# wavelab/libwave

Hardware: AMD Instinct MI355X
Metric: point-cloud registrations/sec (1M<->1M pts, ICP) (higher is better)
Workload: dtype f32

## Files before the change

libwave_amd/csrc/wm_nn.hip:

```cpp
#include "wm_nn_scan.hpp"

namespace wm {

template <int STATS, bool BAL, bool COST = false>
__global__ void __launch_bounds__(64) __attribute__((amdgpu_waves_per_eu(5, 5)))
    k_nn_grid(const LevelsDev *__restrict__ lv, const float4 *__restrict__ src, unsigned n,
              IcpDevState *__restrict__ st, float thr_d2, unsigned long long *__restrict__ keys,
              float4 *__restrict__ match_pt, const float4 *__restrict__ tgt_orig,
              float r_light_cells, float lane_lf, float coop_lf, float r0_cells, unsigned chunk_sz,
              double *__restrict__ partials, unsigned *__restrict__ cost_out,
              unsigned long long *__restrict__ phase_out, long long *__restrict__ bins) {
    const unsigned lane = threadIdx.x & 63u;
    const unsigned row = chunk_sz ? xcd_remap_chunked(blockIdx.x, chunk_sz) : xcd_remap(blockIdx.x, gridDim.x);
    const unsigned i = row * 64u + lane;
    const bool active = i < n;
    const unsigned ic = min(i, n - 1u);
    const float4 p_e = src[ic];
    const unsigned long long prev_e = keys[ic];
    const float4 tp_e = match_pt[ic];
    if (st->done) return;
    unsigned cost = 0;
    unsigned long long prof[3] = {0ull, 0ull, 0ull};
    const unsigned long long prof_start = COST ? clock64() : 0ull;
    __shared__ uint2 s_runs[BAL ? 1 : kRowChunk * 64];
    __shared__ BalHolder<BAL> s_hold;
    const int L = lv->n;
    const int L_levels = L;
    float hl[kMaxLevels];
#pragma unroll
    for (int k = 0; k < kMaxLevels; ++k) hl[k] = lv->g[k < L ? k : 0].h;
    const float h0 = hl[0];
    const float rmax = sqrtf(thr_d2) * 1.0001f + 1e-6f;
    const float r_light = r_light_cells * h0;
    const bool have_prev = st->have_prev != 0;
    float qx = 0.f, qy = 0.f, qz = 0.f, r = 0.f;
    float bqx = 0.f, bqy = 0.f, bqz = 0.f;
    unsigned long long best = make_key(thr_d2, kNoIdx);
    unsigned long long seeded = best;
    bool heavy = false;
    bool mine = active;
    unsigned long long prev = ~0ull;
    float4 tp = make_float4(0.f, 0.f, 0.f, 0.f);
    if (active) {
        if (have_prev) {
            prev = prev_e;
            tp = tp_e;
        }
        xform(st->Tf, p_e, qx, qy, qz);
        if (st->slab_on && !(qx >= st->slab_lo && qx < st->slab_hi)) mine = false;
    }
    if (mine) {
        r = r0_cells * h0;
        if (prev != ~0ull) {
            const unsigned pidx = (unsigned) prev;
            r = rmax;
            if (pidx != kNoIdx) {
                const float d2b = canon_d2(qx, qy, qz, tp);
                if (d2b <= thr_d2) {
                    best = seeded = make_key(d2b, pidx);
                    bqx = tp.x;
                    bqy = tp.y;
                    bqz = tp.z;
                    r = fmaxf(sqrtf(d2b) * 1.0001f + 1e-6f, 0.05f * h0);
                }
            }
        }
        r = fminf(r, rmax);
        heavy = r > r_light;
    }
    const unsigned long long prof_pro = COST ? clock64() : 0ull;
    if constexpr (BAL) {
        BalLds &L = s_hold.v;
        L.q[lane] = make_float4(qx, qy, qz, 0.f);
        L.seeded[lane] = seeded;
        L.bq[0][lane] = bqx;
        L.bq[1][lane] = bqy;
        L.bq[2][lane] = bqz;
        asm volatile("" ::: "memory");
        bool live = mine && !heavy;
        for (int pass = 0; pass < 32 && __ballot(live) != 0ull; ++pass) {
            const int l = nn_level_for(hl, L_levels, lane_lf, r);
            const unsigned long long lv_mask = __ballot(live);
            const int l0 = __builtin_amdgcn_readlane(l, __ffsll((long long) lv_mask) - 1);
            float margin;
            if (__ballot(live && l != l0) == 0ull) {
                const GridDev g = lv->g[l0];
                best = scan_box_bal<COST, kBalRowChunk>(g, live, qx, qy, qz, r, best, &margin, L, lane, have_prev, g.pts, cost, prof);
            } else {
                const GridDev g = lv->g[l];
                L.base[lane] = (unsigned long long) g.pts;
                best = scan_box_bal<COST, kBalRowChunk>(g, live, qx, qy, qz, r, best, &margin, L, lane, have_prev, nullptr, cost, prof);
            }
            if (live) {
                if constexpr (COST) cost += 1u << 24;
                const float bd2 = __uint_as_float((unsigned) (best >> 32));
                if (nn_certified(margin, bd2, thr_d2)) {
                    live = false;
                } else {
                    r = nn_grow_radius(best, bd2, r, rmax);
                    heavy = r > r_light;
                    live = !heavy;
                }
            }
        }
    } else if (mine) {
        for (int pass = 0; !heavy && pass < 32; ++pass) {
            int l = 0;
            while (l < L - 1 && lv->g[l].h < lane_lf * r) ++l;
            const GridDev g = lv->g[l];
            float margin;
            best = scan_box<COST>(g, qx, qy, qz, r, best, &margin, s_runs, lane, have_prev, cost);
            if constexpr (COST) cost += 1u << 24;
            const float bd2 = __uint_as_float((unsigned) (best >> 32));
            if (nn_certified(margin, bd2, thr_d2)) break;
            r = nn_grow_radius(best, bd2, r, rmax);
            heavy = r > r_light;
        }
    }
    const unsigned long long prof_pass = COST ? clock64() : 0ull;
    unsigned long long todo = __ballot(heavy);
    const unsigned n_heavy = __popcll(todo);
    float seed = 0.f;
    while (todo) {
        const int sl = __ffsll((long long) todo) - 1;
        todo &= todo - 1;
        const float ux = rl_f(qx, sl), uy = rl_f(qy, sl), uz = rl_f(qz, sl);
        float ur = rl_f(r, sl);
        unsigned long long ub = ((unsigned long long) rl_u((unsigned) (best >> 32), sl) << 32) |
                                rl_u((unsigned) best, sl);
        if ((unsigned) ub == kNoIdx && seed > ur) ur = fminf(seed, rmax);
        for (int pass = 0; pass < 64; ++pass) {
            int l = 0;
            while (l < L - 1 && lv->g[l].h < coop_lf * ur) ++l;
            const GridDev g = lv->g[l];
            float margin;
            ub = coop_scan_box(g, ux, uy, uz, ur, ub, lane, &margin);
            const float bd2 = __uint_as_float((unsigned) (ub >> 32));
            if (nn_certified(margin, bd2, thr_d2)) break;
            if (ur >= rmax) break;
            ur = nn_grow_radius(ub, bd2, ur, rmax);
        }
        seed = ((unsigned) ub != kNoIdx) ? 1.25f * sqrtf(__uint_as_float((unsigned) (ub >> 32))) : ur;
        if ((int) lane == sl) best = ub;
    }
    const unsigned lane_e = __builtin_amdgcn_mbcnt_hi(~0u, __builtin_amdgcn_mbcnt_lo(~0u, 0u));
    const unsigned i_e = BAL ? row * 64u + lane_e : i;
    if constexpr (BAL) {
        asm volatile("" ::: "memory");
        BalLds &L = s_hold.v;
        seeded = L.seeded[lane_e];
        bqx = L.bq[0][lane_e];
        bqy = L.bq[1][lane_e];
        bqz = L.bq[2][lane_e];
    }
    if (mine) {
        st_u64(&keys[i_e], best);
        if (best != seeded && (unsigned) best != kNoIdx) {
            const f4v c = ((gp_f4) tgt_orig)[(unsigned) best];
            bqx = c.x;
            bqy = c.y;
            bqz = c.z;
        }
        if (!(best == seeded && (unsigned) best != kNoIdx))
            st_f4(&match_pt[i_e], bqx, bqy, bqz, __uint_as_float((unsigned) best));
    }
    if (lane == 0 && n_heavy) atomicAdd(&st->queue_count[1], n_heavy);
    const unsigned long long prof_store = COST ? clock64() : 0ull;
    if constexpr (COST) {
        if (active) cost_out[i_e] = mine ? (cost | (heavy ? 0x80000000u : 0u)) : 0u;
    }
    if constexpr (STATS >= 0) {
        double a[kAcc];
        icp_terms<STATS>(a, mine, (unsigned) best != kNoIdx, qx, qy, qz, bqx, bqy, bqz,
                         __uint_as_float((unsigned) (best >> 32)),
                         (unsigned) best != (unsigned) seeded && (i_e & st->changed_mask) == 0u);
        acc_halve<kAcc, 32>(a, lane);
        const int comp = acc_comp_of_lane(lane);
        if (comp >= 0) {
            if (bins) bins_add(bins, row % (unsigned) kBinCount, (unsigned) comp, a[0]);
            else st_f64(&partials[(size_t) row * kAcc + comp], a[0]);
        }
    }
    if constexpr (COST) {
        if (lane_e == 0 && phase_out) {
            const unsigned long long t_end = clock64();
            atomicAdd(&phase_out[0], prof[0]);
            atomicAdd(&phase_out[1], prof[1]);
            atomicAdd(&phase_out[2], prof[2]);
            atomicAdd(&phase_out[3], prof_pro - prof_start);
            atomicAdd(&phase_out[4], prof_pass - prof_pro);
            atomicAdd(&phase_out[5], prof_store - prof_pass);
            atomicAdd(&phase_out[6], t_end - prof_store);
            atomicAdd(&phase_out[7], 1ull);
        }
    }
}

constexpr int kBruteTile = 1024;

__global__ void __launch_bounds__(kBlock) k_init_keys(unsigned long long *keys, unsigned n,
                                                       const IcpDevState *st, float thr_d2) {
    if (st->done) return;
    const unsigned i = blockIdx.x * kBlock + threadIdx.x;
    if (i < n) keys[i] = make_key(thr_d2, kNoIdx);
}

__global__ void __launch_bounds__(kBlock)
    k_nn_brute(const float4 *__restrict__ tgt, unsigned m, const float4 *__restrict__ src,
               unsigned n, const IcpDevState *__restrict__ st, float thr_d2,
               unsigned long long *__restrict__ keys) {
    if (st->done) return;
    __shared__ float4 tile[kBruteTile];
    const unsigned i = blockIdx.x * kBlock + threadIdx.x;
    const unsigned per = (m + gridDim.y - 1) / gridDim.y;
    const unsigned m0 = blockIdx.y * per, m1 = min(m0 + per, m);
    float qx = 0, qy = 0, qz = 0;
    if (i < n) xform(st->Tf, src[i], qx, qy, qz);
    const bool mine = !(st->slab_on && !(qx >= st->slab_lo && qx < st->slab_hi));
    unsigned long long best = make_key(thr_d2, kNoIdx);
    for (unsigned t0 = m0; t0 < m1; t0 += kBruteTile) {
        const unsigned cnt = min((unsigned) kBruteTile, m1 - t0);
        __syncthreads();
        for (unsigned k = threadIdx.x; k < cnt; k += kBlock) tile[k] = tgt[t0 + k];
        __syncthreads();
        for (unsigned k = 0; k < cnt; ++k) {
            const float4 t = tile[k];
            const unsigned long long key = make_key(canon_d2(qx, qy, qz, t), __float_as_uint(t.w));
            best = key < best ? key : best;
        }
    }
    if (i < n && mine && best < make_key(thr_d2, kNoIdx)) atomicMin(&keys[i], best);
}

__global__ void __launch_bounds__(kBlock)
    k_fill_match(const unsigned long long *__restrict__ keys, unsigned n,
                 const float4 *__restrict__ tgt, const IcpDevState *__restrict__ st,
                 float4 *__restrict__ match_pt) {
    if (st->done) return;
    const unsigned i = blockIdx.x * kBlock + threadIdx.x;
    if (i >= n) return;
    const unsigned idx = (unsigned) keys[i];
    match_pt[i] = idx == kNoIdx ? make_float4(0.f, 0.f, 0.f, __uint_as_float(kNoIdx)) : tgt[idx];
}

static float threshold_below(double max_corr, bool strict) {
    const double m2 = max_corr * max_corr;
    if (!(m2 < 3.0e38)) return 3.0e38f;
    float f = (float) m2;
    if (strict ? (double) f >= m2 : (double) f > m2) f = nextafterf(f, 0.0f);
    return f;
}
float threshold_d2(double max_corr) { return threshold_below(max_corr, false); }
float threshold_d2_strict(double max_corr) { return threshold_below(max_corr, true); }

int nn_sums_target(wm_ctx *ctx, int stats_mode, bool use_bins, unsigned blocks, long long **bins, unsigned *rows_out) {
    *bins = nullptr;
    if (stats_mode >= 0 && use_bins) {
        if (!ctx->bins.p) return WM_ERR_STATE;
        *bins = ctx->bins.as<long long>();
    } else if (stats_mode >= 0) {
        WM_HIP(ctx, ctx->partials.reserve((size_t) blocks * kAcc * sizeof(double)));
        if (rows_out) *rows_out = blocks;
    }
    return WM_OK;
}

template <int STATS, bool BAL, bool COST = false>
static void launch_nn_grid_t(wm_ctx *ctx, unsigned blocks, float thr_d2, unsigned xcd_chunk, long long *bins = nullptr) {
    hipLaunchKernelGGL(HIP_KERNEL_NAME(k_nn_grid<STATS, BAL, COST>), dim3(blocks), dim3(64), 0, ctx->stream,
                       ctx->d_levels.as<LevelsDev>(), ctx->src_sorted.as<float4>(), (unsigned) ctx->n_src,
                       ctx->d_state.as<IcpDevState>(), thr_d2, ctx->keys.as<unsigned long long>(),
                       ctx->match_pt.as<float4>(), ctx->tgt_orig.as<float4>(), ctx->tune_r_light,
                       ctx->tune_lane_lf, ctx->tune_coop_lf, ctx->tune_r0, xcd_chunk, ctx->partials.as<double>(),
                       ctx->cost_log.p ? ctx->cost_log.as<unsigned>() + (size_t) ctx->cost_log_iter * ctx->n_src : nullptr,
                       ctx->phase_log.p ? ctx->phase_log.as<unsigned long long>() + 8 * (size_t) ctx->cost_log_iter : nullptr, bins);
}

int launch_nn_grid(wm_ctx *ctx, float thr_d2, hipEvent_t ev0, hipEvent_t ev1, hipEvent_t ev2,
                   int stats_mode, unsigned *rows_out, bool use_bins) {
    const unsigned n = (unsigned) ctx->n_src;
    if (rows_out) *rows_out = 0;
    if (n == 0) return WM_OK;
    unsigned blocks = (n + 63u) / 64u;
    blocks = (blocks + 7u) & ~7u;
    unsigned xcd_chunk = 0;
    if (ctx->tune_xcd_chunk > 0 && blocks >= 32u * (unsigned) ctx->tune_xcd_chunk) {
        xcd_chunk = (unsigned) ctx->tune_xcd_chunk;
        const unsigned m = 8u * xcd_chunk;
        blocks = (blocks + m - 1u) / m * m;
    }
    long long *bins = nullptr;
    const int rc = nn_sums_target(ctx, stats_mode, use_bins, blocks, &bins, rows_out);
    if (rc != WM_OK) return rc;
    const bool bal = ctx->tune_nn_balanced && ctx->n_tgt_input < (1u << 26) - 8u;
    if (ev0) WM_HIP(ctx, hipEventRecord(ev0, ctx->stream));
    if (stats_mode == WM_ICP_SVD && ctx->cost_log.p && ctx->cost_log_iter < ctx->cost_log_cap) {
        if (bal) launch_nn_grid_t<WM_ICP_SVD, true, true>(ctx, blocks, thr_d2, xcd_chunk, bins);
        else launch_nn_grid_t<WM_ICP_SVD, false, true>(ctx, blocks, thr_d2, xcd_chunk, bins);
        ctx->cost_log_iter++;
    } else if (stats_mode < 0) {
        if (bal) launch_nn_grid_t<-1, true>(ctx, blocks, thr_d2, xcd_chunk);
        else launch_nn_grid_t<-1, false>(ctx, blocks, thr_d2, xcd_chunk);
    } else if (stats_mode == WM_ICP_SVD) {
        if (bal) launch_nn_grid_t<WM_ICP_SVD, true>(ctx, blocks, thr_d2, xcd_chunk, bins);
        else launch_nn_grid_t<WM_ICP_SVD, false>(ctx, blocks, thr_d2, xcd_chunk, bins);
    } else {
        if (bal) launch_nn_grid_t<WM_ICP_GN6, true>(ctx, blocks, thr_d2, xcd_chunk, bins);
        else launch_nn_grid_t<WM_ICP_GN6, false>(ctx, blocks, thr_d2, xcd_chunk, bins);
    }
    if (ev1) WM_HIP(ctx, hipEventRecord(ev1, ctx->stream));
    if (ev2) WM_HIP(ctx, hipEventRecord(ev2, ctx->stream));
    WM_HIP(ctx, hipGetLastError());
    return WM_OK;
}

int launch_nn_brute(wm_ctx *ctx, float thr_d2, hipEvent_t ev0, hipEvent_t ev1) {
    const unsigned n = (unsigned) ctx->n_src, m = (unsigned) ctx->n_tgt_input;
    if (n == 0) return WM_OK;
    const IcpDevState *st = ctx->d_state.as<IcpDevState>();
    unsigned long long *keys = ctx->keys.as<unsigned long long>();
    const unsigned bx = (n + kBlock - 1) / kBlock;
    unsigned splits = 1;
    if (m > 0) {
        splits = (2048 + bx - 1) / bx;
        const unsigned max_splits = (m + kBruteTile - 1) / kBruteTile;
        if (splits > max_splits) splits = max_splits;
        if (splits < 1) splits = 1;
    }
    if (ev0) WM_HIP(ctx, hipEventRecord(ev0, ctx->stream));
    hipLaunchKernelGGL(k_init_keys, dim3(bx), dim3(kBlock), 0, ctx->stream, keys, n, st, thr_d2);
    if (m > 0)
        hipLaunchKernelGGL(k_nn_brute, dim3(bx, splits), dim3(kBlock), 0, ctx->stream,
                           ctx->tgt_orig.as<float4>(), m, ctx->src_sorted.as<float4>(), n, st,
                           thr_d2, keys);
    hipLaunchKernelGGL(k_fill_match, dim3(bx), dim3(kBlock), 0, ctx->stream, keys, n,
                       ctx->tgt_orig.as<float4>(), st, ctx->match_pt.as<float4>());
    if (ev1) WM_HIP(ctx, hipEventRecord(ev1, ctx->stream));
    WM_HIP(ctx, hipGetLastError());
    return WM_OK;
}

}
```

libwave_amd/csrc/wm_nn_scan.hpp:

```cpp
#pragma once
#include "wm_internal.hpp"
#include "wm_icp_step.hpp"
#include "wm_bins.hpp"
#include "wm_wave.hpp"

namespace wm {

__device__ __forceinline__ unsigned long long make_key(float d2, unsigned idx) {
    return ((unsigned long long) __float_as_uint(d2) << 32) | idx;
}

__device__ __forceinline__ float canon_d2(float qx, float qy, float qz, const float4 &t) {
    const float dx = qx - t.x, dy = qy - t.y, dz = qz - t.z;
    return __fadd_rn(__fadd_rn(__fmul_rn(dx, dx), __fmul_rn(dy, dy)), __fmul_rn(dz, dz));
}

__device__ __forceinline__ void xform(const float *T, const float4 &p, float &x, float &y,
                                      float &z) {
    x = __fadd_rn(__fadd_rn(__fadd_rn(__fmul_rn(T[0], p.x), __fmul_rn(T[1], p.y)),
                            __fmul_rn(T[2], p.z)), T[3]);
    y = __fadd_rn(__fadd_rn(__fadd_rn(__fmul_rn(T[4], p.x), __fmul_rn(T[5], p.y)),
                            __fmul_rn(T[6], p.z)), T[7]);
    z = __fadd_rn(__fadd_rn(__fadd_rn(__fmul_rn(T[8], p.x), __fmul_rn(T[9], p.y)),
                            __fmul_rn(T[10], p.z)), T[11]);
}

__device__ __forceinline__ unsigned xcd_remap(unsigned b, unsigned nblocks) {
    const unsigned per = (nblocks + 7u) / 8u;
    return (b & 7u) * per + (b >> 3);
}
__device__ __forceinline__ unsigned xcd_remap_chunked(unsigned b, unsigned S) {
    const unsigned x = b & 7u, l = b >> 3;
    const unsigned chunk = l / S;
    return (chunk * 8u + x) * S + (l - chunk * S);
}

typedef float f4v __attribute__((ext_vector_type(4)));
typedef const __attribute__((address_space(1))) f4v *gp_f4;
typedef const __attribute__((address_space(1))) unsigned *gp_u32;
__device__ __forceinline__ float4 ldp(const float4 *p, size_t j) {
    const f4v v = ((gp_f4) p)[j];
    return make_float4(v.x, v.y, v.z, v.w);
}
__device__ __forceinline__ unsigned ldc(const unsigned *p, size_t j) { return ((gp_u32) p)[j]; }
__device__ __forceinline__ void st_f4(float4 *p, float x, float y, float z, float w) {
    f4v v = {x, y, z, w};
    __builtin_nontemporal_store(v, (f4v *) p);
}
__device__ __forceinline__ void st_u64(unsigned long long *p, unsigned long long v) { __builtin_nontemporal_store(v, p); }
__device__ __forceinline__ void st_f64(double *p, double v) { __builtin_nontemporal_store(v, p); }
__device__ __forceinline__ float canon_d2v(float qx, float qy, float qz, const f4v &t) {
    return canon_d2(qx, qy, qz, make_float4(t.x, t.y, t.z, t.w));
}

__device__ __forceinline__ unsigned long long scan_run(const float4 *__restrict__ pts, unsigned s,
                                                       unsigned e, float qx, float qy, float qz,
                                                       unsigned long long best) {
    for (unsigned j = s; j < e; j += 4) {
        const gp_f4 p = (gp_f4) pts + j;
        const f4v t0 = p[0], t1 = p[1], t2 = p[2], t3 = p[3];
        const unsigned long long k0 = make_key(canon_d2v(qx, qy, qz, t0), __float_as_uint(t0.w));
        const unsigned long long k1 = make_key(canon_d2v(qx, qy, qz, t1), __float_as_uint(t1.w));
        const unsigned long long k2 = make_key(canon_d2v(qx, qy, qz, t2), __float_as_uint(t2.w));
        const unsigned long long k3 = make_key(canon_d2v(qx, qy, qz, t3), __float_as_uint(t3.w));
        const unsigned long long a = k0 < k1 ? k0 : k1, b = k2 < k3 ? k2 : k3;
        const unsigned long long m = a < b ? a : b;
        best = m < best ? m : best;
    }
    return best;
}

constexpr int kRowChunk = 6;
constexpr int kLayeredRows = 18;
template <bool COST>
__device__ __forceinline__ unsigned long long scan_box(const GridDev &g, float qx, float qy,
                                                       float qz, float r, unsigned long long best,
                                                       float *margin, uint2 *runs, unsigned lane,
                                                       bool allow_layered, unsigned &cost) {
    const float big = 4.0e6f;
    const float fx = fminf(fmaxf((qx - g.ox) * g.inv_h, -big), big);
    const float fy = fminf(fmaxf((qy - g.oy) * g.inv_h, -big), big);
    const float fz = fminf(fmaxf((qz - g.oz) * g.inv_h, -big), big);
    const float rc = r * g.inv_h + g.slack;
    const int x0 = (int) floorf(fx - rc), x1 = (int) floorf(fx + rc);
    const int y0 = (int) floorf(fy - rc), y1 = (int) floorf(fy + rc);
    const int z0 = (int) floorf(fz - rc), z1 = (int) floorf(fz + rc);
    const float mx = fminf(fx - (float) x0, (float) (x1 + 1) - fx);
    const float my = fminf(fy - (float) y0, (float) (y1 + 1) - fy);
    const float mz = fminf(fz - (float) z0, (float) (z1 + 1) - fz);
    *margin = (fminf(mx, fminf(my, mz)) - g.slack) * g.h;
    const int xa = max(x0, 0), xb = min(x1, g.nx - 1);
    const int ya = max(y0, 0), yb = min(y1, g.ny - 1);
    const int za = max(z0, 0), zb = min(z1, g.nz - 1);
    if (xa > xb || ya > yb || za > zb) return best;
    auto lookup_and_walk = [&](const unsigned (&a0)[kRowChunk], const unsigned (&a1)[kRowChunk]) {
        unsigned rs[kRowChunk], re[kRowChunk];
#pragma unroll
        for (int u = 0; u < kRowChunk; ++u) {
            rs[u] = ldc(g.cell_start, a0[u]);
            re[u] = ldc(g.cell_start, a1[u]);
        }
        unsigned cnt = 0;
        if constexpr (COST) cost += 1u << 16;
#pragma unroll
        for (int u = 0; u < kRowChunk; ++u)
            if (re[u] > rs[u]) runs[cnt++ * 64u + lane] = make_uint2(rs[u], re[u]);
        unsigned idx = 0, j = 0, e = 0;
        if (cnt) {
            const uint2 run = runs[lane];
            j = run.x;
            e = run.y;
        }
        while (j < e) {
            const gp_f4 p = (gp_f4) g.pts + j;
            const f4v t0 = p[0], t1 = p[1], t2 = p[2], t3 = p[3];
            const unsigned long long k0 = make_key(canon_d2v(qx, qy, qz, t0), __float_as_uint(t0.w));
            const unsigned long long k1 = make_key(canon_d2v(qx, qy, qz, t1), __float_as_uint(t1.w));
            const unsigned long long k2 = make_key(canon_d2v(qx, qy, qz, t2), __float_as_uint(t2.w));
            const unsigned long long k3 = make_key(canon_d2v(qx, qy, qz, t3), __float_as_uint(t3.w));
            const unsigned long long a = k0 < k1 ? k0 : k1, b = k2 < k3 ? k2 : k3;
            const unsigned long long m = a < b ? a : b;
            best = m < best ? m : best;
            j += 4;
            if constexpr (COST) cost += 1u;
            if (j >= e && ++idx < cnt) {
                const uint2 run = runs[idx * 64u + lane];
                j = run.x;
                e = run.y;
            }
        }
    };
    const bool layered =
        allow_layered && __popcll(__ballot((yb - ya + 1) * (zb - za + 1) > kLayeredRows)) >= 8;
    if (layered) {
        for (int kz = 0;; ++kz) {
            const int zz = za + kz;
            const bool zact = zz <= zb;
            if (__ballot(zact) == 0ull) break;
            const float Rb =
                __builtin_amdgcn_sqrtf(__uint_as_float((unsigned) (best >> 32))) * g.inv_h * 1.00001f;
            const float lim = Rb + g.slack;
            const float lim2 = lim * lim, c0 = Rb * Rb + 2.f * g.slack * lim;
            const float rz = fmaxf(fmaxf((float) zz - fz, fz - (float) (zz + 1)), 0.f);
            const float rz2 = rz * rz;
            const float hy = __builtin_amdgcn_sqrtf(fmaxf(lim2 - rz2, 0.f)) * 1.00001f;
            const bool zin = zact && !(rz2 > lim2);
            const int yl = zin ? max(ya, __float2int_rd(fy - hy)) : 1;
            const int yh = zin ? min(yb, __float2int_rd(fy + hy)) : 0;
            const unsigned basez = (unsigned) zz * g.ny * g.nx;
            for (int y0 = yl; __ballot(y0 <= yh) != 0ull; y0 += kRowChunk) {
                unsigned a0[kRowChunk], a1[kRowChunk];
#pragma unroll
                for (int u = 0; u < kRowChunk; ++u) {
                    const int yy = y0 + u;
                    const float yf = (float) yy;
                    const float ry = fmaxf(fmaxf(yf - fy, fy - (yf + 1.f)), 0.f);
                    const float rho2 = ry * ry + rz2;
                    const float hx = __builtin_amdgcn_sqrtf(fmaxf(c0 - rho2, 0.f)) * 1.00001f + g.slack;
                    const int xl = max(xa, __float2int_rd(fx - hx)), xh = min(xb, __float2int_rd(fx + hx));
                    const bool ok = yy <= yh && !(rho2 > lim2) && xl <= xh;
                    const unsigned base = basez + (unsigned) yy * g.nx;
                    a0[u] = ok ? base + xl : 0u;
                    a1[u] = ok ? base + xh + 1 : 0u;
                }
                lookup_and_walk(a0, a1);
            }
        }
        return best;
    }
    int yy = ya, zz = za;
    while (zz <= zb) {
        const float Rb =
            __builtin_amdgcn_sqrtf(__uint_as_float((unsigned) (best >> 32))) * g.inv_h * 1.00001f;
        const float lim = Rb + g.slack;
        const float lim2 = lim * lim, c0 = Rb * Rb + 2.f * g.slack * lim;
        unsigned a0[kRowChunk], a1[kRowChunk];
#pragma unroll
        for (int u = 0; u < kRowChunk; ++u) {
            const float ry = fmaxf(fmaxf((float) yy - fy, fy - (float) (yy + 1)), 0.f);
            const float rz = fmaxf(fmaxf((float) zz - fz, fz - (float) (zz + 1)), 0.f);
            const float rho2 = ry * ry + rz * rz;
            const float hx = __builtin_amdgcn_sqrtf(fmaxf(c0 - rho2, 0.f)) * 1.00001f + g.slack;
            const int xl = max(xa, __float2int_rd(fx - hx)), xh = min(xb, __float2int_rd(fx + hx));
            const bool ok = zz <= zb && !(rho2 > lim2) && xl <= xh;
            const unsigned base = ((unsigned) zz * g.ny + yy) * g.nx;
            a0[u] = ok ? base + xl : 0u;
            a1[u] = ok ? base + xh + 1 : 0u;
            const bool wrap = yy >= yb;
            yy = wrap ? ya : yy + 1;
            zz += wrap;
        }
        lookup_and_walk(a0, a1);
    }
    return best;
}

__device__ __forceinline__ unsigned long long scan_run_bound(const float4 *__restrict__ pts, unsigned s, unsigned e,
                                                             float qx, float qy, float qz, unsigned long long best,
                                                             unsigned &second) {
    for (unsigned j = s; j < e; j += 4) {
        const gp_f4 p = (gp_f4) pts + j;
        const f4v t[4] = {p[0], p[1], p[2], p[3]};
#pragma unroll
        for (int u = 0; u < 4; ++u) {
            const unsigned long long k = make_key(canon_d2v(qx, qy, qz, t[u]), __float_as_uint(t[u].w));
            if (k < best) {
                second = min(second, (unsigned) (best >> 32));
                best = k;
            } else if (k != best) {
                second = min(second, (unsigned) (k >> 32));
            }
        }
    }
    return best;
}

__device__ __forceinline__ unsigned long long wave_min_u64(unsigned long long v) {
#pragma unroll
    for (int off = 32; off > 0; off >>= 1) {
        const unsigned long long o = __shfl_xor(v, off);
        v = o < v ? o : v;
    }
    return v;
}

__device__ __forceinline__ float rl_f(float v, int lane) {
    return __int_as_float(__builtin_amdgcn_readlane(__float_as_int(v), lane));
}
__device__ __forceinline__ unsigned rl_u(unsigned v, int lane) {
    return (unsigned) __builtin_amdgcn_readlane((int) v, lane);
}

constexpr int kBalCap = 1024;
constexpr int kBalRowChunk = 3;
struct BalLds {
    unsigned items[kBalCap + 1];
    float4 q[64];
    unsigned long long base[64];
    unsigned long long best[64];
    unsigned long long seeded[64];
    float bq[3][64];
};

__device__ __forceinline__ unsigned wave_incl_scan(unsigned v) {
    v += (unsigned) __builtin_amdgcn_update_dpp(0, (int) v, 0x111, 0xf, 0xf, true);
    v += (unsigned) __builtin_amdgcn_update_dpp(0, (int) v, 0x112, 0xf, 0xf, true);
    v += (unsigned) __builtin_amdgcn_update_dpp(0, (int) v, 0x114, 0xf, 0xf, true);
    v += (unsigned) __builtin_amdgcn_update_dpp(0, (int) v, 0x118, 0xf, 0xf, true);
    v += (unsigned) __builtin_amdgcn_update_dpp(0, (int) v, 0x142, 0xa, 0xf, false);
    v += (unsigned) __builtin_amdgcn_update_dpp(0, (int) v, 0x143, 0xc, 0xf, false);
    return v;
}

template <bool B>
struct BalHolder {
    BalLds v;
};
template <>
struct BalHolder<false> {
    int unused;
};

struct Bound {
    unsigned second;
    float pad;
    unsigned *lds;
    float4 *win;
    bool ok;
    __device__ __forceinline__ float prune_r(unsigned long long best) const {
        const float b = __builtin_amdgcn_sqrtf(__uint_as_float((unsigned) (best >> 32))) * 1.00001f + pad;
        return fminf(b, __builtin_amdgcn_sqrtf(__uint_as_float(second)) * 1.00001f);
    }
};

template <bool BOUND>
__device__ __forceinline__ void pooled_rounds(BalLds &L, const unsigned *items, unsigned T, unsigned lane,
                                              const float4 *ubase, Bound *bnd) {
    for (unsigned k0 = 0; k0 < T; k0 += 64u) {
        const unsigned k = k0 + lane;
        if (k < T) {
            const unsigned it = items[k];
            const unsigned owner = it >> 26, j = it & 0x3FFFFFFu;
            const float4 q = L.q[owner];
            const gp_f4 p = (gp_f4) (ubase ? ubase : (const float4 *) L.base[owner]) + j;
            const f4v t0 = p[0], t1 = p[1], t2 = p[2], t3 = p[3];
            const float d0 = canon_d2v(q.x, q.y, q.z, t0), d1 = canon_d2v(q.x, q.y, q.z, t1);
            const float d2 = canon_d2v(q.x, q.y, q.z, t2), d3 = canon_d2v(q.x, q.y, q.z, t3);
            const unsigned m = min(min(__float_as_uint(d0), __float_as_uint(d1)), min(__float_as_uint(d2), __float_as_uint(d3)));
            if (m <= __float_as_uint(q.w)) {
                const unsigned long long k0_ = make_key(d0, __float_as_uint(t0.w)), k1_ = make_key(d1, __float_as_uint(t1.w));
                const unsigned long long k2_ = make_key(d2, __float_as_uint(t2.w)), k3_ = make_key(d3, __float_as_uint(t3.w));
                const unsigned long long a = k0_ < k1_ ? k0_ : k1_, b = k2_ < k3_ ? k2_ : k3_;
                if constexpr (BOUND) {
                    const unsigned long long mn = a < b ? a : b;
                    const unsigned u0 = __float_as_uint(d0), u1 = __float_as_uint(d1), u2 = __float_as_uint(d2),
                                   u3 = __float_as_uint(d3);
                    const unsigned lo01 = min(u0, u1), hi01 = max(u0, u1), lo23 = min(u2, u3), hi23 = max(u2, u3);
                    const unsigned sec = min(max(lo01, lo23), min(hi01, hi23));
                    const unsigned long long old = atomicMin(&L.best[owner], mn);
                    unsigned push = sec;
                    if (old != mn) push = min(push, (unsigned) ((old > mn ? old : mn) >> 32));
                    atomicMin(&bnd->lds[owner], push);
                    if (old > mn && bnd->win) {
                        const f4v c = mn == k0_ ? t0 : (mn == k1_ ? t1 : (mn == k2_ ? t2 : t3));
                        bnd->win[owner] = make_float4(c.x, c.y, c.z, c.w);
                    }
                } else {
                    atomicMin(&L.best[owner], a < b ? a : b);
                }
            }
        }
    }
}

template <bool COST, int RC, bool BOUND = false>
__device__ __forceinline__ void balanced_walk(BalLds &L, const unsigned (&rs)[RC],
                                              const unsigned (&re)[RC], unsigned lane,
                                              const float4 *pts, const float4 *ubase, float qx, float qy,
                                              float qz, unsigned long long &best, unsigned &cost,
                                              unsigned long long *prof, Bound *bnd = nullptr) {
    const unsigned long long prof_t0 = COST ? clock64() : 0ull;
    unsigned len[RC], t = 0, longest = 0;
#pragma unroll
    for (int u = 0; u < RC; ++u) {
        len[u] = (unsigned) max((int) (re[u] - rs[u]), 0);
        t += (len[u] + 3u) >> 2;
        longest = max(longest, len[u]);
    }
    const unsigned incl = wave_incl_scan(t);
    const unsigned T = rl_u(incl, 63);
    if (T == 0u) return;
    if constexpr (COST) cost += t;
    if (T > (unsigned) kBalCap) {
        if constexpr (BOUND) {
#pragma unroll
            for (int u = 0; u < RC; ++u) best = scan_run_bound(pts, rs[u], re[u], qx, qy, qz, best, bnd->second);
        } else {
#pragma unroll
            for (int u = 0; u < RC; ++u) best = scan_run(pts, rs[u], re[u], qx, qy, qz, best);
        }
        return;
    }
    unsigned off = incl - t;
    const unsigned tag = lane << 26;
    if (__ballot(longest > 8u) == 0ull) {
#pragma unroll
        for (int u = 0; u < RC; ++u) {
            L.items[len[u] > 0u ? off : (unsigned) kBalCap] = tag | rs[u];
            L.items[len[u] > 4u ? off + 1u : (unsigned) kBalCap] = tag | (rs[u] + 4u);
            off += (len[u] + 3u) >> 2;
        }
    } else {
#pragma unroll
        for (int u = 0; u < RC; ++u)
            for (unsigned j = rs[u]; j < re[u]; j += 4u) L.items[off++] = tag | j;
    }
    L.best[lane] = best;
    if constexpr (BOUND) {
        const float pr = bnd->prune_r(best);
        bnd->lds[lane] = bnd->second;
        reinterpret_cast<unsigned *>(&L.q[lane])[3] = __float_as_uint(pr * pr);
    } else {
        reinterpret_cast<unsigned *>(&L.q[lane])[3] = (unsigned) (best >> 32);
    }
    __builtin_amdgcn_wave_barrier();
    pooled_rounds<BOUND>(L, L.items, T, lane, ubase, bnd);
    __builtin_amdgcn_wave_barrier();
    best = L.best[lane];
    if constexpr (BOUND) bnd->second = bnd->lds[lane];
    if constexpr (COST) {
        prof[0] += clock64() - prof_t0;
        prof[1] += (T + 63u) / 64u;
        prof[2] += 1;
    }
}

template <bool COST, int RC, bool BOUND = false>
__device__ __forceinline__ unsigned long long scan_box_bal(const GridDev &g, bool live, float qx, float qy,
                                                           float qz, float r, unsigned long long best,
                                                           float *margin, BalLds &L, unsigned lane,
                                                           bool allow_layered, const float4 *ubase,
                                                           unsigned &cost, unsigned long long *prof, Bound *bnd = nullptr) {
    const float big = 4.0e6f;
    const float fx = fminf(fmaxf((qx - g.ox) * g.inv_h, -big), big);
    const float fy = fminf(fmaxf((qy - g.oy) * g.inv_h, -big), big);
    const float fz = fminf(fmaxf((qz - g.oz) * g.inv_h, -big), big);
    const float rc = r * g.inv_h + g.slack;
    const int x0 = (int) floorf(fx - rc), x1 = (int) floorf(fx + rc);
    const int y0 = (int) floorf(fy - rc), y1 = (int) floorf(fy + rc);
    const int z0 = (int) floorf(fz - rc), z1 = (int) floorf(fz + rc);
    const float mx = fminf(fx - (float) x0, (float) (x1 + 1) - fx);
    const float my = fminf(fy - (float) y0, (float) (y1 + 1) - fy);
    const float mz = fminf(fz - (float) z0, (float) (z1 + 1) - fz);
    *margin = (fminf(mx, fminf(my, mz)) - g.slack) * g.h;
    const int xa = max(x0, 0), xb = min(x1, g.nx - 1);
    const int ya = max(y0, 0), yb = min(y1, g.ny - 1);
    const int za = max(z0, 0), zb = min(z1, g.nz - 1);
    const bool has = live && !(xa > xb || ya > yb || za > zb);
    auto lookup_and_walk = [&](const unsigned (&a0)[RC], const unsigned (&a1)[RC]) {
        unsigned rs[RC], re[RC];
#pragma unroll
        for (int u = 0; u < RC; ++u) {
            rs[u] = ldc(g.cell_start, a0[u]);
            re[u] = ldc(g.cell_start, a1[u]);
        }
        if constexpr (COST) cost += has ? 1u << 16 : 0u;
        balanced_walk<COST, RC, BOUND>(L, rs, re, lane, g.pts, ubase, qx, qy, qz, best, cost, prof, bnd);
    };
    auto ball_r = [&]() -> float {
        if constexpr (BOUND) return bnd->prune_r(best) * g.inv_h * 1.00001f;
        else return __builtin_amdgcn_sqrtf(__uint_as_float((unsigned) (best >> 32))) * g.inv_h * 1.00001f;
    };
    const bool layered =
        allow_layered && __popcll(__ballot(has && (yb - ya + 1) * (zb - za + 1) > kLayeredRows)) >= 8;
    if (layered) {
        for (int kz = 0;; ++kz) {
            const int zz = za + kz;
            const bool zact = has && zz <= zb;
            if (__ballot(zact) == 0ull) break;
            const float Rb = ball_r();
            const float lim = Rb + g.slack;
            const float lim2 = lim * lim, c0 = Rb * Rb + 2.f * g.slack * lim;
            const float rz = fmaxf(fmaxf((float) zz - fz, fz - (float) (zz + 1)), 0.f);
            const float rz2 = rz * rz;
            const float hy = __builtin_amdgcn_sqrtf(fmaxf(lim2 - rz2, 0.f)) * 1.00001f;
            const bool zin = zact && !(rz2 > lim2);
            const int yl = zin ? max(ya, __float2int_rd(fy - hy)) : 1;
            const int yh = zin ? min(yb, __float2int_rd(fy + hy)) : 0;
            const unsigned basez = (unsigned) zz * g.ny * g.nx;
            for (int yc = yl; __ballot(yc <= yh) != 0ull; yc += RC) {
                unsigned a0[RC], a1[RC];
#pragma unroll
                for (int u = 0; u < RC; ++u) {
                    const int yy = yc + u;
                    const float yf = (float) yy;
                    const float ry = fmaxf(fmaxf(yf - fy, fy - (yf + 1.f)), 0.f);
                    const float rho2 = ry * ry + rz2;
                    const float hx = __builtin_amdgcn_sqrtf(fmaxf(c0 - rho2, 0.f)) * 1.00001f + g.slack;
                    const int xl = max(xa, __float2int_rd(fx - hx)), xh = min(xb, __float2int_rd(fx + hx));
                    const bool ok = yy <= yh && !(rho2 > lim2) && xl <= xh;
                    const unsigned base = basez + (unsigned) yy * g.nx;
                    a0[u] = ok ? base + xl : 0u;
                    a1[u] = ok ? base + xh + 1 : 0u;
                }
                lookup_and_walk(a0, a1);
            }
        }
        return best;
    }
    int yy = ya, zz = has ? za : zb + 1;
    while (__ballot(zz <= zb) != 0ull) {
        const float Rb = ball_r();
        const float lim = Rb + g.slack;
        const float lim2 = lim * lim, c0 = Rb * Rb + 2.f * g.slack * lim;
        unsigned a0[RC], a1[RC];
#pragma unroll
        for (int u = 0; u < RC; ++u) {
            const float ry = fmaxf(fmaxf((float) yy - fy, fy - (float) (yy + 1)), 0.f);
            const float rz = fmaxf(fmaxf((float) zz - fz, fz - (float) (zz + 1)), 0.f);
            const float rho2 = ry * ry + rz * rz;
            const float hx = __builtin_amdgcn_sqrtf(fmaxf(c0 - rho2, 0.f)) * 1.00001f + g.slack;
            const int xl = max(xa, __float2int_rd(fx - hx)), xh = min(xb, __float2int_rd(fx + hx));
            const bool ok = zz <= zb && !(rho2 > lim2) && xl <= xh;
            const unsigned base = ((unsigned) zz * g.ny + yy) * g.nx;
            a0[u] = ok ? base + xl : 0u;
            a1[u] = ok ? base + xh + 1 : 0u;
            const bool wrap = yy >= yb;
            yy = wrap ? ya : yy + 1;
            zz += (wrap && zz <= zb) ? 1 : 0;
        }
        lookup_and_walk(a0, a1);
    }
    return best;
}

constexpr unsigned kRowPool = 128, kRowsPerLane = 16, kRowTrips = 512;
struct RowLds {
    unsigned trips[kRowTrips];
    unsigned map[kRowPool];
    int box[5][64];
};
static_assert(sizeof(RowLds) <= sizeof(unsigned) * (kBalCap + 1), "RowLds overlays BalLds::items");

__device__ __forceinline__ bool scan_box_rows(const GridDev &g, bool live, float qx, float qy, float qz, float r,
                                              unsigned long long &best, float *margin, BalLds &L, unsigned lane,
                                              Bound *bnd) {
    const float big = 4.0e6f;
    const float fx = fminf(fmaxf((qx - g.ox) * g.inv_h, -big), big);
    const float fy = fminf(fmaxf((qy - g.oy) * g.inv_h, -big), big);
    const float fz = fminf(fmaxf((qz - g.oz) * g.inv_h, -big), big);
    const float rc = r * g.inv_h + g.slack;
    const int x0 = (int) floorf(fx - rc), x1 = (int) floorf(fx + rc);
    const int y0 = (int) floorf(fy - rc), y1 = (int) floorf(fy + rc);
    const int z0 = (int) floorf(fz - rc), z1 = (int) floorf(fz + rc);
    const int xa = max(x0, 0), xb = min(x1, g.nx - 1);
    const int ya = max(y0, 0), yb = min(y1, g.ny - 1);
    const int za = max(z0, 0), zb = min(z1, g.nz - 1);
    const bool has = live && !(xa > xb || ya > yb || za > zb);
    const int wy = yb - ya + 1;
    const unsigned nrows = has ? (unsigned) (wy * (zb - za + 1)) : 0u;
    const unsigned incl = wave_incl_scan(nrows);
    const unsigned R = rl_u(incl, 63);
    if (R > kRowPool || __ballot(nrows > kRowsPerLane) != 0ull) return false;
    {
        const float mx = fminf(fx - (float) x0, (float) (x1 + 1) - fx);
        const float my = fminf(fy - (float) y0, (float) (y1 + 1) - fy);
        const float mz = fminf(fz - (float) z0, (float) (z1 + 1) - fz);
        *margin = (fminf(mx, fminf(my, mz)) - g.slack) * g.h;
    }
    if (R == 0u) return true;
    RowLds &W = *reinterpret_cast<RowLds *>(L.items);
    const float pr = bnd->prune_r(best);
    L.best[lane] = best;
    bnd->lds[lane] = bnd->second;
    reinterpret_cast<unsigned *>(&L.q[lane])[3] = __float_as_uint(pr * pr);
    W.box[0][lane] = xa;
    W.box[1][lane] = xb;
    W.box[2][lane] = ya;
    W.box[3][lane] = za;
    W.box[4][lane] = wy;
    for (unsigned k = 0, off = incl - nrows; k < nrows; ++k) W.map[off + k] = lane | (k << 8);
    __builtin_amdgcn_wave_barrier();
    unsigned ttot = 0;
    bool fits = true;
    for (unsigned b0 = 0; b0 < R; b0 += 64u) {
        unsigned rs = 0, re = 0, owner = 0;
        if (b0 + lane < R) {
            const unsigned m = W.map[b0 + lane];
            owner = m & 63u;
            const int k = (int) (m >> 8), wyo = W.box[4][owner];
            const int yy = W.box[2][owner] + k % wyo, zz = W.box[3][owner] + k / wyo;
            const float4 q = L.q[owner];
            const float ofx = fminf(fmaxf((q.x - g.ox) * g.inv_h, -big), big);
            const float ofy = fminf(fmaxf((q.y - g.oy) * g.inv_h, -big), big);
            const float ofz = fminf(fmaxf((q.z - g.oz) * g.inv_h, -big), big);
            const float Rb = __builtin_amdgcn_sqrtf(q.w) * g.inv_h * 1.00003f;
            const float lim = Rb + g.slack;
            const float lim2 = lim * lim, c0 = Rb * Rb + 2.f * g.slack * lim;
            const float ry = fmaxf(fmaxf((float) yy - ofy, ofy - (float) (yy + 1)), 0.f);
            const float rz = fmaxf(fmaxf((float) zz - ofz, ofz - (float) (zz + 1)), 0.f);
            const float rho2 = ry * ry + rz * rz;
            const float hx = __builtin_amdgcn_sqrtf(fmaxf(c0 - rho2, 0.f)) * 1.00001f + g.slack;
            const int xl = max(W.box[0][owner], __float2int_rd(ofx - hx)), xh = min(W.box[1][owner], __float2int_rd(ofx + hx));
            if (!(rho2 > lim2) && xl <= xh) {
                const unsigned base = ((unsigned) zz * g.ny + yy) * g.nx;
                rs = ldc(g.cell_start, base + xl);
                re = ldc(g.cell_start, base + xh + 1);
            }
        }
        const unsigned len = (unsigned) max((int) (re - rs), 0), t = (len + 3u) >> 2;
        const unsigned incl2 = wave_incl_scan(t);
        const unsigned Tb = rl_u(incl2, 63);
        if (Tb > kRowTrips) {
            fits = false;
            break;
        }
        if (ttot + Tb > kRowTrips) {
            __builtin_amdgcn_wave_barrier();
            pooled_rounds<true>(L, W.trips, ttot, lane, g.pts, bnd);
            __builtin_amdgcn_wave_barrier();
            ttot = 0;
        }
        unsigned o = ttot + incl2 - t;
        for (unsigned j = rs; j < re; j += 4u) W.trips[o++] = (owner << 26) | j;
        ttot += Tb;
    }
    __builtin_amdgcn_wave_barrier();
    if (fits) pooled_rounds<true>(L, W.trips, ttot, lane, g.pts, bnd);
    __builtin_amdgcn_wave_barrier();
    best = L.best[lane];
    bnd->second = bnd->lds[lane];
    return fits;
}

__device__ __forceinline__ unsigned long long coop_scan_box(const GridDev &g, float qx, float qy,
                                                            float qz, float r,
                                                            unsigned long long best, unsigned lane,
                                                            float *margin, unsigned *second_out = nullptr,
                                                            float pad = 0.f) {
    const float fx = (qx - g.ox) * g.inv_h, fy = (qy - g.oy) * g.inv_h, fz = (qz - g.oz) * g.inv_h;
    const float rc = r * g.inv_h + g.slack;
    const float big = 4.0e6f;
    const int x0 = (int) floorf(fminf(fmaxf(fx - rc, -big), big));
    const int x1 = (int) floorf(fminf(fmaxf(fx + rc, -big), big));
    const int y0 = (int) floorf(fminf(fmaxf(fy - rc, -big), big));
    const int y1 = (int) floorf(fminf(fmaxf(fy + rc, -big), big));
    const int z0 = (int) floorf(fminf(fmaxf(fz - rc, -big), big));
    const int z1 = (int) floorf(fminf(fmaxf(fz + rc, -big), big));
    const float mx = fminf(fx - (float) x0, (float) (x1 + 1) - fx);
    const float my = fminf(fy - (float) y0, (float) (y1 + 1) - fy);
    const float mz = fminf(fz - (float) z0, (float) (z1 + 1) - fz);
    *margin = (fminf(mx, fminf(my, mz)) - g.slack) * g.h;
    const int xa = max(x0, 0), xb = min(x1, g.nx - 1);
    const int ya = max(y0, 0), yb = min(y1, g.ny - 1);
    const int za = max(z0, 0), zb = min(z1, g.nz - 1);
    if (xa > xb || ya > yb || za > zb) return best;
    const int cy = (int) floorf(fminf(fmaxf(fy, -big), big));
    const int cz = (int) floorf(fminf(fmaxf(fz, -big), big));
    const int wy = yb - ya + 1;
    const int nrows = wy * (zb - za + 1);
    const float bd2 = __uint_as_float((unsigned) (best >> 32));
    const float Rb = (__builtin_amdgcn_sqrtf(bd2) + pad) * g.inv_h * 1.00001f;
    unsigned long long mine = best;
    unsigned mine2 = 0x7F800000u;
    for (int k0 = 0; k0 < nrows; k0 += 64) {
        const int k = k0 + (int) lane;
        unsigned s = 0, e = 0;
        if (k < nrows) {
            const int yy = ya + k % wy, zz = za + k / wy;
            const float ry = yy > cy ? (float) yy - fy : (yy < cy ? fy - (float) (yy + 1) : 0.f);
            const float rz = zz > cz ? (float) zz - fz : (zz < cz ? fz - (float) (zz + 1) : 0.f);
            const float rho2 = ry * ry + rz * rz;
            const float lim = Rb + g.slack;
            if (!(rho2 > lim * lim)) {
                const float hx2 = fmaxf(Rb * Rb - rho2 + 2.f * g.slack * lim, 0.f);
                const float hx = __builtin_amdgcn_sqrtf(hx2) * 1.00001f + g.slack;
                const int xl = max(xa, (int) floorf(fminf(fmaxf(fx - hx, -big), big)));
                const int xh = min(xb, (int) floorf(fminf(fmaxf(fx + hx, -big), big)));
                if (xl <= xh) {
                    const size_t base = ((size_t) zz * g.ny + yy) * g.nx;
                    s = ldc(g.cell_start, base + xl);
                    e = ldc(g.cell_start, base + xh + 1);
                }
            }
        }
        unsigned long long rows = __ballot(e > s);
        while (rows) {
            const int rl = __ffsll((long long) rows) - 1;
            rows &= rows - 1;
            const unsigned rs = rl_u(s, rl), re = rl_u(e, rl);
            for (unsigned j = rs + lane; j < re; j += 128u) {
                const float4 t0 = ldp(g.pts, j);
                const float4 t1 = ldp(g.pts, j + 64u < re ? j + 64u : j);
                const unsigned long long a = make_key(canon_d2(qx, qy, qz, t0), __float_as_uint(t0.w));
                const unsigned long long b = make_key(canon_d2(qx, qy, qz, t1), __float_as_uint(t1.w));
                const unsigned long long m = a < b ? a : b;
                if (second_out) {
                    const unsigned long long hi = a < b ? b : a;
                    if (m < mine) {
                        mine2 = min(mine2, min((unsigned) (mine >> 32), hi != m ? (unsigned) (hi >> 32) : 0x7F800000u));
                    } else {
                        if (m != mine) mine2 = min(mine2, (unsigned) (m >> 32));
                        if (hi != mine && hi != m) mine2 = min(mine2, (unsigned) (hi >> 32));
                    }
                }
                mine = m < mine ? m : mine;
            }
        }
    }
    const unsigned long long all = wave_min_u64(mine);
    if (second_out) {
        unsigned v = mine != all ? min(mine2, (unsigned) (mine >> 32)) : mine2;
#pragma unroll
        for (int off = 32; off > 0; off >>= 1) v = min(v, (unsigned) __shfl_xor((int) v, off));
        *second_out = min(*second_out, v);
    }
    return all;
}

__device__ __forceinline__ bool nn_certified(float margin, float bd2, float thr_d2) {
    return margin > 0.f && (bd2 <= margin * margin || thr_d2 <= margin * margin);
}
__device__ __forceinline__ float nn_grow_radius(unsigned long long best, float bd2, float r, float rmax, float pad = 0.f) {
    const float rn = ((unsigned) best != kNoIdx) ? sqrtf(bd2) * 1.0001f + 1e-6f + pad : 2.0f * r;
    return fminf(fmaxf(rn, 1.25f * r), rmax);
}
__device__ __forceinline__ int nn_level_for(const float (&hl)[kMaxLevels], int levels, float lf, float r) {
    int l = 0;
#pragma unroll
    for (int k = 0; k < kMaxLevels - 1; ++k) l += (k < levels - 1 && hl[k] < lf * r) ? 1 : 0;
    return l;
}
constexpr int kCertWaves = 4;
__device__ __forceinline__ void chunk_query(unsigned e, const unsigned (&cum)[kCertWaves + 1], unsigned &w, unsigned &k) {
    w = (e >= cum[1] ? 1u : 0u) + (e >= cum[2] ? 1u : 0u) + (e >= cum[3] ? 1u : 0u);
    k = e - (w == 0u ? cum[0] : (w == 1u ? cum[1] : (w == 2u ? cum[2] : cum[3])));
}
__device__ __forceinline__ double add_wave_rows(const double (&rows)[kCertWaves][kAcc], unsigned c) {
    double t = rows[0][c];
#pragma unroll
    for (int w = 1; w < kCertWaves; ++w) t += rows[w][c];
    return t;
}


constexpr double kChangedUnit = 1.0 / 16777216.0;
template <int STATS>
__device__ __forceinline__ void icp_terms(double (&a)[kAcc], bool mine, bool matched, float qx, float qy, float qz,
                                          float bqx, float bqy, float bqz, float d2, bool changed = false) {
#pragma unroll
    for (int k = 0; k < kAcc; ++k) a[k] = 0.0;
    if (mine) {
        a[17] = changed ? 1.0 + kChangedUnit : 1.0;
        if (matched) {
            const double px = qx, py = qy, pz = qz, tx = bqx, ty = bqy, tz = bqz;
            a[0] = 1.0;
            a[1] = px;
            a[2] = py;
            a[3] = pz;
            if constexpr (STATS == WM_ICP_SVD) {
                a[4] = tx;
                a[5] = ty;
                a[6] = tz;
                a[7] = tx * px;
                a[8] = tx * py;
                a[9] = tx * pz;
                a[10] = ty * px;
                a[11] = ty * py;
                a[12] = ty * pz;
                a[13] = tz * px;
                a[14] = tz * py;
                a[15] = tz * pz;
            } else {
                const double rx = px - tx, ry = py - ty, rz = pz - tz;
                a[4] = py * py + pz * pz;
                a[5] = -px * py;
                a[6] = -px * pz;
                a[7] = px * px + pz * pz;
                a[8] = -py * pz;
                a[9] = px * px + py * py;
                a[10] = rx;
                a[11] = ry;
                a[12] = rz;
                a[13] = py * rz - pz * ry;
                a[14] = pz * rx - px * rz;
                a[15] = px * ry - py * rx;
            }
            a[16] = (double) d2;
        }
    }
}

}
```

Baseline: 276.5.

## Early-exit empty rows, use fast sqrt intrinsic, branchless SVD accumulation terms

Wavefronts whose entire row lies past n now exit early after zeroing their partial-sum slot, instead of running the full search prologue. Several sqrtf calls in the radius logic become __builtin_amdgcn_sqrtf, which avoids the correctly rounded sqrt sequence but may return slightly less accurate radii. The SVD branch of icp_terms computes all accumulator terms with selects instead of a zero-init loop plus branches, reducing divergence and register traffic. The radius changes feed only search bounds, which are padded, so matches should be unaffected unless the small rounding changes certification decisions.

```diff
diff --git a/libwave_amd/csrc/wm_nn.hip b/libwave_amd/csrc/wm_nn.hip
--- a/libwave_amd/csrc/wm_nn.hip
+++ b/libwave_amd/csrc/wm_nn.hip
@@ -19,6 +19,13 @@
     const unsigned long long prev_e = keys[ic];
     const float4 tp_e = match_pt[ic];
     if (st->done) return;
+    if (row * 64u >= n) {
+        if constexpr (STATS >= 0) {
+            const int comp0 = acc_comp_of_lane(lane);
+            if (!bins && comp0 >= 0) st_f64(&partials[(size_t) row * kAcc + comp0], 0.0);
+        }
+        return;
+    }
     unsigned cost = 0;
     unsigned long long prof[3] = {0ull, 0ull, 0ull};
     const unsigned long long prof_start = COST ? clock64() : 0ull;
@@ -30,7 +37,7 @@
 #pragma unroll
     for (int k = 0; k < kMaxLevels; ++k) hl[k] = lv->g[k < L ? k : 0].h;
     const float h0 = hl[0];
-    const float rmax = sqrtf(thr_d2) * 1.0001f + 1e-6f;
+    const float rmax = __builtin_amdgcn_sqrtf(thr_d2) * 1.0001f + 1e-6f;
     const float r_light = r_light_cells * h0;
     const bool have_prev = st->have_prev != 0;
     float qx = 0.f, qy = 0.f, qz = 0.f, r = 0.f;
@@ -61,7 +68,7 @@
                     bqx = tp.x;
                     bqy = tp.y;
                     bqz = tp.z;
-                    r = fmaxf(sqrtf(d2b) * 1.0001f + 1e-6f, 0.05f * h0);
+                    r = fmaxf(__builtin_amdgcn_sqrtf(d2b) * 1.0001f + 1e-6f, 0.05f * h0);
                 }
             }
         }
@@ -97,7 +104,7 @@
                 if (nn_certified(margin, bd2, thr_d2)) {
                     live = false;
                 } else {
-                    r = nn_grow_radius(best, bd2, r, rmax);
+                    r = nn_grow_radius<true>(best, bd2, r, rmax);
                     heavy = r > r_light;
                     live = !heavy;
                 }
@@ -113,7 +120,7 @@
             if constexpr (COST) cost += 1u << 24;
             const float bd2 = __uint_as_float((unsigned) (best >> 32));
             if (nn_certified(margin, bd2, thr_d2)) break;
-            r = nn_grow_radius(best, bd2, r, rmax);
+            r = nn_grow_radius<true>(best, bd2, r, rmax);
             heavy = r > r_light;
         }
     }
@@ -138,9 +145,9 @@
             const float bd2 = __uint_as_float((unsigned) (ub >> 32));
             if (nn_certified(margin, bd2, thr_d2)) break;
             if (ur >= rmax) break;
-            ur = nn_grow_radius(ub, bd2, ur, rmax);
-        }
-        seed = ((unsigned) ub != kNoIdx) ? 1.25f * sqrtf(__uint_as_float((unsigned) (ub >> 32))) : ur;
+            ur = nn_grow_radius<true>(ub, bd2, ur, rmax);
+        }
+        seed = ((unsigned) ub != kNoIdx) ? 1.25f * __builtin_amdgcn_sqrtf(__uint_as_float((unsigned) (ub >> 32))) : ur;
         if ((int) lane == sl) best = ub;
     }
     const unsigned lane_e = __builtin_amdgcn_mbcnt_hi(~0u, __builtin_amdgcn_mbcnt_lo(~0u, 0u));
diff --git a/libwave_amd/csrc/wm_nn_scan.hpp b/libwave_amd/csrc/wm_nn_scan.hpp
--- a/libwave_amd/csrc/wm_nn_scan.hpp
+++ b/libwave_amd/csrc/wm_nn_scan.hpp
@@ -661,8 +661,9 @@
 __device__ __forceinline__ bool nn_certified(float margin, float bd2, float thr_d2) {
     return margin > 0.f && (bd2 <= margin * margin || thr_d2 <= margin * margin);
 }
+template <bool FAST = false>
 __device__ __forceinline__ float nn_grow_radius(unsigned long long best, float bd2, float r, float rmax, float pad = 0.f) {
-    const float rn = ((unsigned) best != kNoIdx) ? sqrtf(bd2) * 1.0001f + 1e-6f + pad : 2.0f * r;
+    const float rn = ((unsigned) best != kNoIdx) ? (FAST ? __builtin_amdgcn_sqrtf(bd2) : sqrtf(bd2)) * 1.0001f + 1e-6f + pad : 2.0f * r;
     return fminf(fmaxf(rn, 1.25f * r), rmax);
 }
 __device__ __forceinline__ int nn_level_for(const float (&hl)[kMaxLevels], int levels, float lf, float r) {
@@ -688,6 +689,30 @@
 template <int STATS>
 __device__ __forceinline__ void icp_terms(double (&a)[kAcc], bool mine, bool matched, float qx, float qy, float qz,
                                           float bqx, float bqy, float bqz, float d2, bool changed = false) {
+    if constexpr (STATS == WM_ICP_SVD) {
+        const bool on = mine && matched;
+        const double px = on ? qx : 0.f, py = on ? qy : 0.f, pz = on ? qz : 0.f;
+        const double tx = on ? bqx : 0.f, ty = on ? bqy : 0.f, tz = on ? bqz : 0.f;
+        a[0] = on ? 1.0 : 0.0;
+        a[1] = px;
+        a[2] = py;
+        a[3] = pz;
+        a[4] = tx;
+        a[5] = ty;
+        a[6] = tz;
+        a[7] = tx * px;
+        a[8] = tx * py;
+        a[9] = tx * pz;
+        a[10] = ty * px;
+        a[11] = ty * py;
+        a[12] = ty * pz;
+        a[13] = tz * px;
+        a[14] = tz * py;
+        a[15] = tz * pz;
+        a[16] = (double) (on ? d2 : 0.f);
+        a[17] = mine ? (changed ? 1.0 + kChangedUnit : 1.0) : 0.0;
+        return;
+    }
 #pragma unroll
     for (int k = 0; k < kAcc; ++k) a[k] = 0.0;
     if (mine) {
```

Result: no change. 276.9 (median of 2 runs) (+0.1%).
